# beecave-homelab/VibeVoice-ROCm

Measured on AMD Instinct MI355X. Metric: audio-sec/s, higher is better.
Workload: dtype bf16; 1 GPU; cfg2: VibeVoice-1.5B shapes, 1 speaker(s) x 203-frame voice prompt, 330-token prompt, 225 frames (30.0 s audio), CFG=2.0, 20 DPM-Solver++ steps, whole generate() incl. voice encode + prefill; global_batch=1, parallelism=replicas x1 (one dialogue per GPU), hipgraph=True

## Files before the change

include/vv_hip.h:

```cpp
#ifndef VV_HIP_H
#define VV_HIP_H

#include <stddef.h>
#include <stdint.h>

#ifdef __cplusplus
extern "C" {
#endif

typedef void* vv_stream_t;

enum { VV_F32 = 0, VV_BF16 = 1, VV_FP8 = 2  };
enum { VV_NF4 = 3 };
enum { VV_WQ_NF4 = 0x100 };
enum { VV_OK = 0, VV_E_ARG = -1, VV_E_HIP = -2, VV_E_UNSUPPORTED = -3 };
enum { VV_PRO_NONE = 0, VV_PRO_RMSNORM = 1, VV_PRO_SILU = 2 };
enum { VV_ACT_NONE = 0, VV_ACT_GELU = 1, VV_ACT_SWIGLU = 2 };
enum { VV_LIN_X_BF16 = 1, VV_LIN_OUT_BF16 = 2, VV_LIN_W_REUSED = 4, VV_LIN_W_FRAG = 8 };

const char* vv_last_error(void);
int vv_abi_version(void);
int vv_tune(const char* key, int value);
int vv_init(void);

// ... 154 lines not shown

size_t vv_block_mid_ws_bytes(int T, int C);
int vv_block_mid(const struct vv_block* b, int wdt, const float* x, float* out, void* ws, int T, int C, float eps, vv_stream_t stream);

typedef struct vv_conv {
  const void* w;
  const float* b;
  int cin, cout, kk, stride, transposed;
  float* state;
} vv_conv;

#define VV_MAX_STAGES 8
typedef struct vv_convnet {
  int wdt, n_stages;
  float eps;
  vv_conv sample[VV_MAX_STAGES];
  int n_blocks[VV_MAX_STAGES];
  const vv_block* blocks[VV_MAX_STAGES];
  vv_conv head;
} vv_convnet;

size_t vv_convnet_ws_bytes(const vv_convnet* net, int64_t t_in, int decoder);
int vv_decoder_forward(const vv_convnet* net, const float* latent, int T, float pre_scale, float pre_bias, float* wav,
                       void* ws, vv_stream_t stream);
int vv_encoder_forward(const vv_convnet* net, const float* wav, int64_t T, float* feat, void* ws, vv_stream_t stream);
int vv_convnet_reset(const vv_convnet* net, vv_stream_t stream);

typedef struct vv_connector { int wdt, din, hidden; const void* fc1; const float* b1; const float* norm_w; const void* fc2; const float* b2; } vv_connector;
int vv_connector_forward(const vv_connector* c, const float* x, int R, float* out, int accumulate, float* ws, vv_stream_t stream);
int vv_connector_pair(const vv_connector* ac, const vv_connector* sem, const float* latent, const float* semfeat, float* out, int64_t ldo,
                      int rows_out, float* ws, vv_stream_t stream);

int vv_graph_begin(vv_stream_t stream);
int vv_graph_end(vv_stream_t stream, void** graph_exec_out);
int vv_graph_launch(void* graph_exec, vv_stream_t stream);
int vv_graph_destroy(void* graph_exec);

typedef struct vv_prof_entry { int m, n, k, dual, wdt, count; double total_ms; } vv_prof_entry;
int vv_prof_begin(int max_records);
int vv_prof_end(vv_prof_entry* out, int max_out, int* n_out);

typedef struct vv_nf4_src {
  const uint8_t* packed;
  const void* absmax;
  const float* quant_map;
  const float* nested_absmax;
  const float* nested_map;
  float nested_offset;
  int nested_blocksize;
  int n, k, blocksize;
} vv_nf4_src;
int vv_nf4_import(const vv_nf4_src* src, void* w, int64_t ldw, int row0, int rows_total, void* cq, float* cs, vv_stream_t stream);

size_t vv_sizeof(const char* struct_name);

#ifdef __cplusplus
}
#endif
#endif
```

vibevoice_rocm_amd/_lib.py:

```python
from __future__ import annotations

import ctypes as C
import os

_HERE = os.path.dirname(os.path.abspath(__file__))
LIB_PATH = os.path.join(_HERE, "libvv_hip.so")

VV_F32, VV_BF16, VV_FP8, VV_NF4 = 0, 1, 2, 3
VV_WQ_NF4 = 0x100
PRO_NONE, PRO_RMSNORM, PRO_SILU = 0, 1, 2
ACT_NONE, ACT_GELU, ACT_SWIGLU = 0, 1, 2
LIN_X_BF16, LIN_OUT_BF16, LIN_W_REUSED, LIN_W_FRAG = 1, 2, 4, 8
VV_MAX_STAGES = 8

vp = C.c_void_p
i64 = C.c_int64


class W8(C.Structure):
    _fields_ = [("q", vp), ("scale", vp)]


class LinArgs(C.Structure):
    _fields_ = [("x", vp), ("ldx", i64), ("m", C.c_int), ("pro", C.c_int), ("norm_w", vp), ("eps", C.c_float),
# ... 68 lines not shown
_STRUCTS = dict(vv_w8=W8, vv_prof_entry=ProfEntry, vv_lin_args=LinArgs, vv_kv=KV, vv_llm_layer=LlmLayer, vv_llm=Llm, vv_head_layer=HeadLayer, vv_head=Head,
                vv_dpm_coef=DpmCoef, vv_block=Block, vv_conv=Conv, vv_convnet=ConvNet, vv_connector=Connector, vv_nf4_src=Nf4Src)

PROTOTYPES = {
    "vv_last_error": (C.c_char_p, []),
    "vv_abi_version": (C.c_int, []),
    "vv_init": (C.c_int, []),
    "vv_tune": (C.c_int, [C.c_char_p, C.c_int]),
    "vv_linear": (C.c_int, [C.POINTER(LinArgs), vp]),
    "vv_rope_table": (C.c_int, [vp, vp, C.c_int, C.c_int, vp, vp]),
    "vv_rope_store": (C.c_int, [vp, i64, C.c_int, C.c_int, C.POINTER(KV), C.c_int, vp, vp, vp, vp]),
    "vv_attn": (C.c_int, [vp, i64, C.c_int, C.c_int, C.POINTER(KV), C.c_int, vp, vp, vp, i64, vp]),
    "vv_attn_decode": (C.c_int, [vp, i64, C.c_int, C.c_int, C.POINTER(KV), C.c_int, vp, vp, vp, i64, vp]),
    "vv_block_mixer": (C.c_int, [vp, vp, C.c_int, C.c_int, vp, C.c_float, vp, vp, vp, vp, vp]),
    "vv_block1d": (C.c_int, [vp, C.c_int, vp, vp, C.c_int, C.c_int, C.c_float, vp]),
    "vv_block_mid_ws_bytes": (C.c_size_t, [C.c_int, C.c_int]),
    "vv_block_mid": (C.c_int, [vp, C.c_int, vp, vp, vp, C.c_int, C.c_int, C.c_float, vp]),
    "vv_conv_ctx": (C.c_int, [vp, vp, C.c_int, C.c_int, C.c_int, vp]),
    "vv_affine": (C.c_int, [vp, C.c_float, C.c_float, vp, i64, vp]),
    "vv_add_rows": (C.c_int, [vp, i64, vp, i64, vp, C.c_int, C.c_int, C.c_int, vp]),
    "vv_add_rows_silu": (C.c_int, [vp, i64, vp, i64, vp, C.c_int, C.c_int, C.c_int, vp]),
    "vv_add_rows_silu_bf16": (C.c_int, [vp, i64, vp, i64, vp, C.c_int, C.c_int, C.c_int, vp]),
    "vv_dpm_proj": (C.c_int, [vp, i64, C.c_float, C.POINTER(DpmCoef), vp, vp, vp, vp, vp, C.c_int, C.c_int, C.c_int, vp, i64, C.c_int, vp, vp]),
    "vv_embed_row": (C.c_int, [vp, C.c_int, i64, vp, vp, vp]),
    "vv_gather_rows": (C.c_int, [vp, C.c_int, i64, C.POINTER(C.c_int), C.c_int, vp, vp]),
    "vv_argmax_ids": (C.c_int, [vp, C.c_int, vp, vp, vp, vp]),
    "vv_cast_rows_bf16": (C.c_int, [vp, i64, C.c_int, C.c_int, C.c_int, vp, C.c_float, vp, i64, vp]),
    "vv_copy_rows": (C.c_int, [vp, i64, vp, i64, C.c_int, C.c_int, vp]),
    "vv_dpm_step": (C.c_int, [vp, i64, C.c_int, C.c_int, C.c_float, C.c_float, C.c_float, C.c_float, C.c_float,
                              C.c_float, C.c_int, vp, vp, vp]),
    "vv_advance_lens": (C.c_int, [vp, vp, C.c_int, C.c_int, vp, vp]),
    "vv_llm_ws_bytes": (C.c_size_t, [C.POINTER(Llm), C.c_int]),
    "vv_llm_forward": (C.c_int, [C.POINTER(Llm), C.POINTER(KV), vp, i64, C.c_int, vp, vp, vp, i64, vp, vp]),
    "vv_llm_tail": (C.c_int, [C.POINTER(Llm), vp, i64, C.c_int, vp, i64, vp, C.c_int, vp, vp, vp, vp, vp, C.c_int, C.c_int, vp, vp]),
    "vv_llm_tail_batch": (C.c_int, [C.POINTER(Llm), vp, i64, C.c_int, vp, i64, vp, C.c_int, vp, vp, vp, vp, vp, C.c_int, C.c_int, vp, vp, vp]),
    "vv_head_ws_bytes": (C.c_size_t, [C.POINTER(Head), C.c_int]),
    "vv_head_ws_bytes_batch": (C.c_size_t, [C.POINTER(Head), C.c_int, C.c_int]),
    "vv_head_sample_batch": (C.c_int, [C.POINTER(Head), vp, i64, vp, i64, vp, C.POINTER(DpmCoef), C.c_int, C.c_float, vp, i64, C.c_int, vp, vp]),
    "vv_head_ws_bytes_batch_sde": (C.c_size_t, [C.POINTER(Head), C.c_int, C.c_int]),
    "vv_head_sample_batch_sde": (C.c_int, [C.POINTER(Head), vp, i64, vp, i64, vp, C.POINTER(DpmCoef), C.c_int, C.c_float, vp, i64, C.c_int, vp, vp, i64, vp]),
    "vv_head_sample": (C.c_int, [C.POINTER(Head), vp, i64, vp, vp, C.POINTER(DpmCoef), C.c_int, C.c_float, vp, vp, vp, vp]),
    "vv_head_forward": (C.c_int, [C.POINTER(Head), vp, vp, vp, C.c_int, vp, vp, vp]),
    "vv_convnet_ws_bytes": (C.c_size_t, [C.POINTER(ConvNet), i64, C.c_int]),
    "vv_decoder_forward": (C.c_int, [C.POINTER(ConvNet), vp, C.c_int, C.c_float, C.c_float, vp, vp, vp]),
    "vv_encoder_forward": (C.c_int, [C.POINTER(ConvNet), vp, i64, vp, vp, vp]),
    "vv_convnet_reset": (C.c_int, [C.POINTER(ConvNet), vp]),
    "vv_connector_forward": (C.c_int, [C.POINTER(Connector), vp, C.c_int, vp, C.c_int, vp, vp]),
    "vv_connector_pair": (C.c_int, [C.POINTER(Connector), C.POINTER(Connector), vp, vp, vp, i64, C.c_int, vp, vp]),
    "vv_graph_begin": (C.c_int, [vp]),
    "vv_graph_end": (C.c_int, [vp, C.POINTER(vp)]),
    "vv_graph_launch": (C.c_int, [vp, vp]),
    "vv_graph_destroy": (C.c_int, [vp]),
    "vv_nf4_import": (C.c_int, [C.POINTER(Nf4Src), vp, i64, C.c_int, C.c_int, vp, vp, vp]),
    "vv_sizeof": (C.c_size_t, [C.c_char_p]),
    "vv_prof_begin": (C.c_int, [C.c_int]),
    "vv_prof_end": (C.c_int, [C.POINTER(ProfEntry), C.c_int, C.POINTER(C.c_int)]),
}


class VVError(RuntimeError):
    pass


_lib = None


def load():
    global _lib
    if _lib is not None:
        return _lib
    import torch
    if not os.path.exists(LIB_PATH):
        raise VVError(f"{LIB_PATH} is missing: build the HIP extension first (python -m vibevoice_rocm_amd.build). "
                      "The MI355X kernels are the only compute path of this package.")
    lib = C.CDLL(LIB_PATH)
    for name, (res, args) in PROTOTYPES.items():
        fn = getattr(lib, name)
        fn.restype = res
        fn.argtypes = args
    for cname, cls in _STRUCTS.items():
        n = lib.vv_sizeof(cname.encode())
        if n != C.sizeof(cls):
            raise VVError(f"ABI mismatch for {cname}: C side {n} bytes, ctypes mirror {C.sizeof(cls)} bytes")
    _lib = lib
    return lib


def check(rc: int, what: str = ""):
    if rc != 0:
        raise VVError(f"{what} failed ({rc}): {load().vv_last_error().decode()}")


def ptr(t) -> int:
    return 0 if t is None else t.data_ptr()
```

vibevoice_rocm_amd/build.py:

```python
from __future__ import annotations

import hashlib
import os
import shutil
import subprocess
import sys

HERE = os.path.dirname(os.path.abspath(__file__))
ROOT = os.path.dirname(HERE)
SRC = [os.path.join(HERE, "csrc", f) for f in ("vv_kernels.hip", "vv_gemv_stream.hip", "vv_gemv_hot.hip", "vv_gemv_rows.hip", "vv_mfma_gemm.hip", "vv_block1d.hip", "vv_convffn.hip",
                                               "vv_fused.hip", "vv_attn_decode.hip", "vv_attn_prefill.hip", "vv_model.hip",
                                               "vv_nf4_import.hip")]
HDR = [os.path.join(ROOT, "include", "vv_hip.h"), os.path.join(HERE, "csrc", "vv_common.h")]
OUT = os.path.join(HERE, "libvv_hip.so")
OBJDIR = os.path.join(HERE, "csrc", "build")
STAMP = os.path.join(HERE, "libvv_hip.stamp")
FLAGS = ["--offload-arch=gfx950", "-O3", "-std=c++17", "-fPIC"]


def find_hipcc() -> str:
    for c in (os.environ.get("HIPCC"), shutil.which("hipcc"), "/opt/rocm/bin/hipcc"):
        if c and os.path.exists(c):
            return c
    raise RuntimeError("hipcc not found (ROCm toolchain required to build the MI355X kernels)")


def _flavour() -> str:
    return hashlib.sha256("\n".join([os.path.basename(s) for s in SRC] + FLAGS).encode()).hexdigest()[:16]


def _check_sources():
    missing = [p for p in SRC + HDR if not os.path.exists(p)]
    if missing:
        raise RuntimeError("missing kernel sources: " + ", ".join(os.path.relpath(p, ROOT) for p in missing))


def up_to_date() -> bool:
    if not os.path.exists(OUT):
        return False
    if not all(os.path.exists(p) for p in SRC + HDR):
        return True
    t = os.path.getmtime(OUT)
    if not all(os.path.getmtime(p) <= t for p in SRC + HDR):
        return False
    try:
        return open(STAMP).read().strip() == _flavour()
    except OSError:
        return False


def _obj(src: str) -> str:
    return os.path.join(OBJDIR, os.path.basename(src) + ".o")


def build(force: bool = False, verbose: bool = True, jobs: int = 6) -> str:
    if not force and up_to_date():
        return OUT
    _check_sources()
    os.makedirs(OBJDIR, exist_ok=True)
    flags = [*FLAGS, "-I" + os.path.join(ROOT, "include"), "-I" + os.path.join(HERE, "csrc")]
    hipcc = find_hipcc()
    hdr_t = max(os.path.getmtime(p) for p in HDR)
    todo = [s for s in SRC if force or not os.path.exists(_obj(s)) or os.path.getmtime(_obj(s)) < max(os.path.getmtime(s), hdr_t)]
# ... 24 lines not shown
```

vibevoice_rocm_amd/csrc/vv_common.h:

```cpp
#ifndef VV_COMMON_H
#define VV_COMMON_H
#include <hip/hip_runtime.h>
#include <stdarg.h>
#include <stdint.h>
#include "vv_hip.h"

int vv_set_error(int code, const char* fmt, ...);

#define VV_CHECK_LAUNCH(name)                                                                    \
  do {                                                                                           \
    hipError_t e_ = hipGetLastError();                                                           \
    if (e_ != hipSuccess) return vv_set_error(VV_E_HIP, "%s: %s", name, hipGetErrorString(e_));  \
  } while (0)

#define VV_TRY(expr)            \
  do {                          \
    int rc_ = (expr);           \
    if (rc_) return rc_;        \
  } while (0)

int vv_launch_gemv_stream(const vv_lin_args& a, hipStream_t s);
struct vv_gemv_hot_shape { const char* name; int m, n, k, dual, pro, mod, bias, gate, res, act, flags; };
extern "C" int vv_gemv_hot_shapes(vv_gemv_hot_shape* out, int cap);
int vv_launch_gemv_hot(const vv_lin_args& a, hipStream_t s);
void vv_gemv_hot_set(int mask);
int vv_launch_gemv_rows(const vv_lin_args& a, float* part, size_t part_floats, int* tickets, size_t n_tickets, hipStream_t s);
size_t vv_gemv_rows_part_floats(int n, int dual);
size_t vv_gemv_rows_tickets(int n);
int vv_gemv_rows_init();
void vv_gemv_rows_set(int on, int blocks, int pers);
int vv_linear_ws(const vv_lin_args* a, const void* f1, const void* f2, float* part, size_t part_floats, int* tickets, size_t n_tickets,
                 vv_stream_t stream, const vv_w8* q1 = nullptr, const vv_w8* q2 = nullptr);
int vv_launch_mfma_gemm(const vv_lin_args& a, hipStream_t s);
int vv_mfma_gemm_init();
int vv_launch_attn_decode(const float* qkv, int64_t ld_qkv, int R, int heads, const vv_kv* kv, int layer, const float2* rope, const int* lens, float* out,
                          int64_t ldo, float* part, int* tickets, int nsplit, int part_cap, hipStream_t s);
int vv_attn_decode_ws(const float* qkv, int64_t ld_qkv, int R, int heads, const vv_kv* kv, int layer, const float* rope_table, const int* lens, float* out,
                      int64_t ldo, float* part, int* tickets, int nsplit, int part_cap, vv_stream_t stream);
int vv_launch_attn_prefill(const float* qkv, int64_t ld_qkv, int R, int heads, const vv_kv* kv, int layer, const int* lens, const int* cache_rows,
                           float* out, int64_t ldo, hipStream_t s);
int vv_head_init_fused(const vv_head* h, const float* noise, float* Xs, float* Ms, float* h0, int64_t ldh, hipStream_t s);
bool vv_head_boundary_supported(const vv_head* h);
int vv_head_boundary_fused(const vv_head* h, const float* hrows, int64_t ldh, const float* shift, const float* scale, int64_t ld_mod, float cfg,
                           const vv_dpm_coef* k, float* Xs, float* Ms, float* h_out, int64_t ldh_out, float* latent_out, hipStream_t s);
int vv_head_boundary_batch(const vv_head* h, const float* hrows, int64_t ldh, const float* shift, const float* scale, int64_t ld_mod, float cfg,
                           const vv_dpm_coef* k, float* Xs, float* Ms, int64_t state_stride, float* h_out, int64_t ldh_out, float* latent_out,
                           int64_t latent_stride, int B, hipStream_t s,
                           const float* nx = nullptr, int64_t nx_stride = 0);
int vv_head_sde_proj_fused(const vv_head* h, const float* sde_noise, int64_t ld_sde, int n_steps, int B, float* NX, hipStream_t s);
int vv_fused_init();
int vv_head_pre_fused(const vv_head* h, const float* cond2, int64_t ld_cond, const float* temb, int n_steps, void* c_bf16, const float* noise,
                      float* Xs, float* Ms, float* h0, int64_t ldh, hipStream_t s);
int vv_launch_connector_pair(const vv_connector* ac, const vv_connector* sem, const float* latent, const float* semfeat, float* out, int64_t ldo, int rows_out,
                             float* ws, hipStream_t s);
int vv_head_modulations_fused(const vv_head* h, const void* c_bf16, int rows, float* const* mod, float* modf, hipStream_t s);
struct vv_conv_ctx_item { float* pad; float* state; int ctx, T, C; const float* dw_w; float* hs; int affine; float scale, bias; };
int vv_conv_ctx_batch(const vv_conv_ctx_item* items, int n, int scatter, hipStream_t s);
int vv_block1d_init();
int vv_launch_block1d(const vv_block& B, int wdt, const float* x, float* out, int T, int C, float eps, hipStream_t s);
void vv_block1d_set_fused(int on);
void vv_block1d_set_blocks(int b);
int vv_convffn_init();
int vv_launch_convffn(const vv_block& B, int wdt, const float* x, float* y, void* hidden, float* hist_new, float* out, int T, int C, float eps,
                      hipStream_t s);
void vv_convffn_set(int on);
int vv_launch_ffn_in_row(const vv_block& B, int wdt, const float* x, float* y, float* hidden, float* hist_new, int C, float eps, hipStream_t s);
void vv_convffn_set_t1(int on);
int vv_launch_ffn_in_row_hs(const vv_block& B, int wdt, const float* x, float* y, float* hidden, float* hist_new, int C, float eps, hipStream_t s);
void vv_convffn_set_t1hs(int on);
void vv_convffn_set_rows(int c, int rows);
void vv_convffn_set_c128(int on);
bool vv_convffn_prefers(int wdt, int T, int C);
int vv_launch_skinny(const vv_lin_args& a, hipStream_t s);
void vv_skinny_set(int on, int min_m, int max_m);
int vv_rmsnorm_rows(const float* x, int64_t ldx, const float* w, float eps, int rows, int n, float* out, int64_t ldo, hipStream_t s);

#ifdef __HIPCC__
__device__ __forceinline__ float vv_gelu_as(float v) {
// ... 24 lines not shown
```

vibevoice_rocm_amd/csrc/vv_convffn.hip:

```cpp
#include <hip/hip_runtime.h>
#include <hip/hip_bf16.h>
#include <stdint.h>

#include "vv_hip.h"
#include "vv_common.h"

namespace {

typedef unsigned short bf16_t;
typedef __bf16 bf16x8 __attribute__((ext_vector_type(8)));
typedef float f32x16 __attribute__((ext_vector_type(16)));
typedef float f32x4 __attribute__((ext_vector_type(4)));
typedef unsigned int u32x4 __attribute__((ext_vector_type(4)));

#ifdef VV_CF_TIMING
__device__ unsigned long long g_cf_t[8];
#define CSTAMP(i) do { if (blockIdx.x == 0 && blockIdx.y == 0 && threadIdx.x == 0) { const long long t_ = wall_clock64(); g_cf_t[i] += (unsigned long long)(t_ - tprev_); tprev_ = t_; } } while (0)
#else
#define CSTAMP(i) do { } while (0)
#endif

constexpr int TR2 = 16;
constexpr int HALO = 6;

// ... 494 lines not shown
#define VV_SK(NSTV, NBV) hipLaunchKernelGGL((skinny_kernel<NSTV, NBV>), grid, dim3(256), 0, s, a.x, a.ldx, a.m, W, a.k, a.bias, a.out, a.ldo)
  switch (a.k) {
    case 128: VV_SK(1, 1); break;
    case 256: VV_SK(2, 1); break;
    case 512: VV_SK(4, 1); break;
    case 1024: VV_SK(8, 1); break;
    case 2048: VV_SK(16, 1); break;
    case 2560: VV_SK(20, 1); break;
    case 5120: VV_SK(20, 2); break;
    default: return 0;
  }
#undef VV_SK
  return 1;
}

int vv_convffn_init() {
#define VV_CF_ATTR(CC, TT)                                                                                                                  \
  { constexpr int nt_ = in_threads<CC>(); constexpr int l_ = (int)InLay<CC, TT, nt_>::LDS;                                                 \
    if (hipFuncSetAttribute(reinterpret_cast<const void*>(&ffn_in_kernel<CC, TT, false, nt_>), hipFuncAttributeMaxDynamicSharedMemorySize, l_) != hipSuccess) \
      return vv_set_error(VV_E_HIP, "vv_convffn_init: cannot raise the LDS limit"); }
  VV_CF_ATTR(128, 16) VV_CF_ATTR(128, 32) VV_CF_ATTR(256, 8) VV_CF_ATTR(256, 16) VV_CF_ATTR(256, 32) VV_CF_ATTR(512, 8) VV_CF_ATTR(512, 16) VV_CF_ATTR(512, 32) VV_CF_ATTR(1024, 8)
#undef VV_CF_ATTR
  {
    constexpr int l1 = (int)InLay<2048, 1, 256>::LDS;
    if (hipFuncSetAttribute(reinterpret_cast<const void*>(&ffn_in_kernel<2048, 1, true, 256>), hipFuncAttributeMaxDynamicSharedMemorySize, l1) != hipSuccess)
      return vv_set_error(VV_E_HIP, "vv_convffn_init: cannot raise the LDS limit");
  }
  return 0;
}

int g_t1 = 1;
void vv_convffn_set_t1(int on) { g_t1 = on; }

int vv_launch_ffn_in_row(const vv_block& B, int wdt, const float* x, float* y, float* hidden, float* hist_new, int C, float eps, hipStream_t s) {
  if (!g_on || !g_t1 || wdt != VV_BF16 || C != 2048 || !B.hist) return 0;
  auto a16 = [](const void* q) { return q && ((uintptr_t)q % 16) == 0; };
  if (!a16(B.w1) || !a16(B.b1) || !a16(B.gamma) || !a16(B.norm_w) || !a16(B.ffn_norm_w) || !a16(B.dw_b) || !a16(B.dw_w) || !a16(x) || !a16(y) ||
      !a16(hidden) || !a16(hist_new) || !a16(B.hist) || x == y)
    return 0;
  constexpr size_t lds = InLay<2048, 1, 256>::LDS;
  hipLaunchKernelGGL((ffn_in_kernel<2048, 1, true, 256>), dim3(4 * 2048 / 32, 1), dim3(256), lds, s, x, y, hidden, hist_new, 1, B, eps);
  return hipGetLastError() == hipSuccess ? 1 : vv_set_error(VV_E_HIP, "vv_convffn: launch failed");
}

int g_t1hs = 1;
void vv_convffn_set_t1hs(int on) { g_t1hs = on; }

int vv_launch_ffn_in_row_hs(const vv_block& B, int wdt, const float* x, float* y, float* hidden, float* hist_new, int C, float eps, hipStream_t s) {
  if (!g_on || !g_t1 || !g_t1hs || wdt != VV_BF16 || C != 2048 || !B.hist || !B.hs || !B.dw_last) return 0;
  auto a16 = [](const void* q) { return q && ((uintptr_t)q % 16) == 0; };
  if (!a16(B.w1) || !a16(B.b1) || !a16(B.gamma) || !a16(B.norm_w) || !a16(B.ffn_norm_w) || !a16(B.dw_b) || !a16(B.dw_last) || !a16(B.hs) || !a16(x) ||
      !a16(y) || !a16(hidden) || !a16(hist_new) || !a16(B.hist) || x == y)
    return 0;
  hipLaunchKernelGGL(ffn_in_row_kernel, dim3(4 * 2048 / 32), dim3(256), 0, s, x, y, hidden, hist_new, B, eps);
  return hipGetLastError() == hipSuccess ? 1 : vv_set_error(VV_E_HIP, "vv_convffn: launch failed");
}

int vv_launch_convffn(const vv_block& B, int wdt, const float* x, float* y, void* hidden, float* hist_new, float* out, int T, int C, float eps,
                      hipStream_t s) {
  if (!g_on || wdt != VV_BF16 || T < 3 || (C != 128 && C != 256 && C != 512 && C != 1024) || (C == 1024 && T > 64)) return 0;
  if (C == 128 ? (!g_c128 || T > 1024) : T > 256) return 0;
  auto a16 = [](const void* q) { return q && ((uintptr_t)q % 16) == 0; };
  if (!a16(B.w1) || !a16(B.w2) || !a16(B.b1) || !B.b2 || !a16(B.gamma) || !B.ffn_gamma || !a16(B.norm_w) || !a16(B.ffn_norm_w) || !a16(B.dw_b) ||
      !a16(B.dw_w) || !a16(x) || !a16(y) || !a16(hidden) || !a16(hist_new) || !out || (B.hist && !a16(B.hist)))
    return 0;
  {
    const uintptr_t xa = (uintptr_t)x, ya = (uintptr_t)y, bytes = (uintptr_t)T * C * 4;
    if (xa < ya + bytes && ya < xa + bytes) return 0;
  }
  if (C == 128) {
    if (g_trv128 == 16) return launch_c<128, 16, 4>(B, x, y, hidden, hist_new, out, T, eps, s);
    return launch_c<128, 32, 4>(B, x, y, hidden, hist_new, out, T, eps, s);
  }
  if (C == 256) {
    if (g_trv256 == 8) return launch_c<256, 8, 4>(B, x, y, hidden, hist_new, out, T, eps, s);
    if (g_trv256 == 16) return launch_c<256, 16, 4>(B, x, y, hidden, hist_new, out, T, eps, s);
    return launch_c<256, 32, 4>(B, x, y, hidden, hist_new, out, T, eps, s);
  }
  if (C == 512) {
    if (g_trv512 == 8) return launch_c<512, 8, 4>(B, x, y, hidden, hist_new, out, T, eps, s);
    if (g_trv512 == 16) return launch_c<512, 16, 4>(B, x, y, hidden, hist_new, out, T, eps, s);
    return launch_c<512, 32, 4>(B, x, y, hidden, hist_new, out, T, eps, s);
  }
  return launch_c<1024, 8, 8>(B, x, y, hidden, hist_new, out, T, eps, s);
}

extern "C" size_t vv_block_mid_ws_bytes(int T, int C) { return (size_t)T * C * 4 + (size_t)T * 4 * C * 2 + (size_t)HALO * C * 4 + 64; }

extern "C" int vv_block_mid(const vv_block* b, int wdt, const float* x, float* out, void* ws, int T, int C, float eps, vv_stream_t stream) {
  if (!b || !x || !out || !ws || T <= 0) return vv_set_error(VV_E_ARG, "vv_block_mid: bad args");
  float* y = reinterpret_cast<float*>(ws);
  char* hidden = reinterpret_cast<char*>(ws) + (size_t)T * C * 4;
  float* hn = reinterpret_cast<float*>(hidden + (size_t)T * 4 * C * 2);
  const int rc = vv_launch_convffn(*b, wdt, x, y, hidden, hn, out, T, C, eps, (hipStream_t)stream);
  if (rc < 0) return rc;
  if (rc == 0) return vv_set_error(VV_E_UNSUPPORTED, "vv_block_mid: shape not covered (C=%d T=%d wdt=%d)", C, T, wdt);
  return 0;
}
```

vibevoice_rocm_amd/csrc/vv_gemv_stream.hip:

```cpp
#include <hip/hip_runtime.h>
#include <stdint.h>

#include "vv_hip.h"
#include "vv_common.h"

namespace {

typedef unsigned short bf16_t;
typedef unsigned int u32x4 __attribute__((ext_vector_type(4)));

__device__ __forceinline__ float wsum(float v) { return vv_wave_sum(v); }
__device__ __forceinline__ float silu1(float v) { return v / (1.0f + expf(-v)); }
__device__ __forceinline__ float gelu1(float v) { return 0.5f * v * (1.0f + erff(v * 0.70710678118654752440f)); }

__device__ __forceinline__ void unpack8(const u32x4 v, float (&o)[8]) {
  o[0] = __uint_as_float(v.x << 16); o[1] = __uint_as_float(v.x & 0xffff0000u);
  o[2] = __uint_as_float(v.y << 16); o[3] = __uint_as_float(v.y & 0xffff0000u);
  o[4] = __uint_as_float(v.z << 16); o[5] = __uint_as_float(v.z & 0xffff0000u);
  o[6] = __uint_as_float(v.w << 16); o[7] = __uint_as_float(v.w & 0xffff0000u);
}

typedef unsigned int u32x2 __attribute__((ext_vector_type(2)));
typedef float f32x2 __attribute__((ext_vector_type(2)));
__device__ __forceinline__ void unpack8_f8(const u32x4 v, float (&o)[8]) {
// ... 551 lines not shown
    case 8: return launch_kus<M, DUAL, 8>(a, s, ku);
    case 16: if constexpr (!DUAL) return launch_kus<M, false, 16>(a, s, ku); else return false;
  }
  return false;
}

bool launch_m8(const vv_lin_args& a, hipStream_t s, int ksplit, int ku) {
  if (ksplit == 1) {
    if (ku == 1) launch_rw<8, false, 1, 1, 1>(a, s); else launch_rw<8, false, 1, 2, 1>(a, s);
    return true;
  }
  switch (ksplit) {
    case 4: launch_rw<8, false, 4, 2, 2>(a, s); return true;
    case 8: launch_rw<8, false, 8, 2, 2>(a, s); return true;
  }
  return false;
}

}

void vv_gemv_stream_set_blocks(int b) { g_blocks_override = b; }
void vv_gemv_stream_set_waves(int w) { g_waves_override = w; }
void vv_gemv_stream_set_opt(int o) { g_opt = o; }
void vv_gemv_stream_set_long(int cap, int ku) { if (cap > 0) g_long_cap = cap; if (ku > 0) g_long_ku = ku; }
void vv_gemv_stream_set_dual_rw(int r) { g_dual_rw = r; }
void vv_gemv_stream_set_small_rw(int r) { g_small_rw = r; }

int vv_launch_gemv_stream(const vv_lin_args& a, hipStream_t s) {
  if ((a.wdt != VV_BF16 && a.wdt != VV_FP8 && a.wdt != VV_NF4) || a.m > 8 || a.k % 8) return 0;
  if (a.wdt == VV_NF4 && (a.m > 2 || a.k % 64 || !a.wscale || (a.w2 && !a.w2scale) || (uintptr_t)a.w % 16 || (a.w2 && (uintptr_t)a.w2 % 16) ||
                          (uintptr_t)a.wscale % 4 || (a.w2 && (uintptr_t)a.w2scale % 4) || (a.flags & VV_LIN_W_FRAG)))
    return 0;
  if (a.wdt == VV_FP8 && (a.m > 2 || !a.wscale || (a.w2 && !a.w2scale) || (uintptr_t)a.w % 8 || (a.w2 && (uintptr_t)a.w2 % 8))) return 0;
  if (a.m > 4) {
    if (a.w2 || a.wdt != VV_BF16) return 0;
    if ((uintptr_t)a.w % 16 || (uintptr_t)a.x % 16 || a.ldx % 4) return 0;
    if (a.norm_w && (uintptr_t)a.norm_w % 16) return 0;
    if (a.mod_scale && ((uintptr_t)a.mod_scale % 16 || (uintptr_t)a.mod_shift % 16 || a.ld_mod % 4)) return 0;
    const int units8 = (a.k + 511) / 512;
    int ks = 0, ku8 = 0;
    for (int w : {1, 4, 8}) {
      if ((units8 + w - 1) / w <= 2) { ks = w; ku8 = (units8 + w - 1) / w; break; }
    }
    if (!ks) return 0;
    if (ks > 1) ku8 = 2;
    return launch_m8(a, s, ks, ku8) ? 1 : 0;
  }
  if (a.wdt == VV_BF16 && ((uintptr_t)a.w % 16 || (a.w2 && (uintptr_t)a.w2 % 16))) return 0;
  if ((uintptr_t)a.x % 16) return 0;
  if (a.m > 1 && a.ldx % 4) return 0;
  if (a.norm_w && (uintptr_t)a.norm_w % 16) return 0;
  if (a.mod_scale && ((uintptr_t)a.mod_scale % 16 || (uintptr_t)a.mod_shift % 16 || a.ld_mod % 4)) return 0;
  if (a.m == 2 && a.wdt == VV_BF16 && vv_launch_gemv_hot(a, s)) return 1;
  const int units = (a.k + 511) / 512;
  const bool dual = a.w2 != nullptr;
  int ksplit = 1, ku = units;
  if (units > ((a.wdt == VV_NF4 && dual) ? 4 : 5)) {
    const int kumax = dual ? 3 : (units > 12 ? g_long_ku : 5);
    ksplit = 0;
    for (int w : {4, 8, 16}) {
      if ((units + w - 1) / w <= kumax) { ksplit = w; ku = (units + w - 1) / w; break; }
    }
    if (!ksplit) return 0;
    if (ku < 2) ku = 2;
  }
  if (a.wdt == VV_NF4 && ksplit > 8) return 0;
  bool ok;
  if (a.m == 1) ok = dual ? launch_ku<1, true>(a, s, ksplit, ku) : launch_ku<1, false>(a, s, ksplit, ku);
  else if (a.m == 2) ok = dual ? launch_ku<2, true>(a, s, ksplit, ku) : launch_ku<2, false>(a, s, ksplit, ku);
  else ok = dual ? launch_ku<4, true>(a, s, ksplit, ku) : launch_ku<4, false>(a, s, ksplit, ku);
  return ok ? 1 : 0;
}
```

vibevoice_rocm_amd/csrc/vv_kernels.hip:

```cpp
#include <hip/hip_runtime.h>
#include <hip/hip_bf16.h>
#include <stdint.h>
#include <stdio.h>
#include <string.h>
#include <math.h>

#include "vv_hip.h"
#include "vv_common.h"

static thread_local char g_err[512] = "";

int vv_set_error(int code, const char* fmt, ...) {
  va_list ap;
  va_start(ap, fmt);
  vsnprintf(g_err, sizeof(g_err), fmt, ap);
  va_end(ap);
  return code;
}

extern "C" const char* vv_last_error(void) { return g_err; }
extern "C" int vv_abi_version(void) { return 6; }
int vv_mixer_init();
extern "C" int vv_init(void) {
  VV_TRY(vv_mixer_init());
  VV_TRY(vv_mfma_gemm_init());
  VV_TRY(vv_block1d_init());
  VV_TRY(vv_convffn_init());
  VV_TRY(vv_gemv_rows_init());
  return vv_fused_init();
}
static float* g_rows_part = nullptr;
static int* g_rows_tk = nullptr;
static const size_t G_ROWS_PART_FLOATS = (size_t)4 << 20, G_ROWS_TICKETS = 4096;
static int rows_scratch(int on) {
  if (on && !g_rows_part) {
    if (hipMalloc(&g_rows_part, G_ROWS_PART_FLOATS * sizeof(float)) != hipSuccess || hipMalloc(&g_rows_tk, G_ROWS_TICKETS * sizeof(int)) != hipSuccess ||
        hipMemset(g_rows_tk, 0, G_ROWS_TICKETS * sizeof(int)) != hipSuccess)
      return vv_set_error(VV_E_HIP, "vv_tune: gemv_rows_scratch allocation failed");
  }
  if (!on && g_rows_part) { (void)hipFree(g_rows_part); (void)hipFree(g_rows_tk); g_rows_part = nullptr; g_rows_tk = nullptr; }
  return 0;
}
void vv_gemv_rows_set_dbg(int d);
void vv_gemv_rows_set_atomic(int on);
void vv_gemv_stream_set_blocks(int b);
void vv_gemv_stream_set_waves(int w);
void vv_gemv_stream_set_opt(int o);
void vv_gemv_stream_set_long(int cap, int ku);
void vv_gemv_stream_set_dual_rw(int r);
void vv_gemv_stream_set_small_rw(int r);
void vv_mfma_set_mt(int mt);
void vv_mfma_set_tiled_rows(int r);
void vv_mfma_set_tiled_bk128(int on);
void vv_mfma_set_tiled_small(int t);
void vv_mfma_set_tiled_dual_bk64(int on);
void vv_mfma_set_tiled_small_dual(int t);
void vv_mfma_set_tiled_small_k(int k);
void vv_mixer_set_rows(int on);
void vv_mfma_set_mt_prefill(int mt);
extern int g_attn_group;
void vv_attn_decode_set_gqa(int on);
void vv_attn_decode_set_gqa_keys(int k);
extern "C" int vv_tune(const char* key, int value) {
  if (key && !strcmp(key, "gemv_long_cap")) { vv_gemv_stream_set_long(value, 0); return 0; }
  if (key && !strcmp(key, "gemv_long_ku")) { vv_gemv_stream_set_long(0, value); return 0; }
  if (key && !strcmp(key, "gemv_blocks")) { vv_gemv_stream_set_blocks(value); return 0; }
  if (key && !strcmp(key, "gemv_waves")) { vv_gemv_stream_set_waves(value); return 0; }
  if (key && !strcmp(key, "gemv_rows")) { vv_gemv_rows_set(value, 0, -1); return 0; }
  if (key && !strcmp(key, "gemv_rows_blocks")) { vv_gemv_rows_set(-1, value, -1); return 0; }
  if (key && !strcmp(key, "gemv_rows_pers")) { vv_gemv_rows_set(-1, 0, value); return 0; }
  if (key && !strcmp(key, "gemv_rows_scratch")) return rows_scratch(value);
  if (key && !strcmp(key, "gemv_rows_dbg")) { vv_gemv_rows_set_dbg(value); return 0; }
  if (key && !strcmp(key, "gemv_rows_atomic")) { vv_gemv_rows_set_atomic(value); return 0; }
  if (key && !strcmp(key, "gemv_opt")) { vv_gemv_stream_set_opt(value); return 0; }
  if (key && !strcmp(key, "gemv_dual_rw")) { vv_gemv_stream_set_dual_rw(value); return 0; }
  if (key && !strcmp(key, "gemv_small_rw")) { vv_gemv_stream_set_small_rw(value); return 0; }
  if (key && !strcmp(key, "gemv_hot")) { vv_gemv_hot_set(value); return 0; }
  if (key && !strcmp(key, "mixer_rows")) { vv_mixer_set_rows(value); return 0; }
  if (key && !strcmp(key, "block1d_fused")) { vv_block1d_set_fused(value); return 0; }
  if (key && !strcmp(key, "block1d_blocks")) { vv_block1d_set_blocks(value); return 0; }
  if (key && !strcmp(key, "convffn")) { vv_convffn_set(value); return 0; }
  if (key && !strcmp(key, "convffn_t1")) { vv_convffn_set_t1(value); return 0; }
  if (key && !strcmp(key, "convffn_t1hs")) { vv_convffn_set_t1hs(value); return 0; }
  if (key && !strcmp(key, "convffn_rows512")) { vv_convffn_set_rows(512, value); return 0; }
  if (key && !strcmp(key, "convffn_rows256")) { vv_convffn_set_rows(256, value); return 0; }
  if (key && !strcmp(key, "convffn_rows128")) { vv_convffn_set_rows(128, value); return 0; }
  if (key && !strcmp(key, "convffn_c128")) { vv_convffn_set_c128(value); return 0; }
  if (key && !strcmp(key, "skinny")) { vv_skinny_set(value, 0, 0); return 0; }
  if (key && !strcmp(key, "skinny_min_m")) { vv_skinny_set(1, value, 0); return 0; }
  if (key && !strcmp(key, "skinny_max_m")) { vv_skinny_set(1, 0, value); return 0; }
  if (key && !strcmp(key, "mfma_tiled_bk128")) { vv_mfma_set_tiled_bk128(value); return 0; }
  if (key && !strcmp(key, "attn_group")) { g_attn_group = value; return 0; }
  if (key && !strcmp(key, "attn_gqa")) { vv_attn_decode_set_gqa(value); return 0; }
  if (key && !strcmp(key, "attn_gqa_keys")) { vv_attn_decode_set_gqa_keys(value); return 0; }
  if (key && !strcmp(key, "mfma_tiled_small_k")) { vv_mfma_set_tiled_small_k(value); return 0; }
  if (key && !strcmp(key, "mfma_tiled_dual_bk64")) { vv_mfma_set_tiled_dual_bk64(value); return 0; }
  if (key && !strcmp(key, "mfma_tiled_small_dual")) { vv_mfma_set_tiled_small_dual(value); return 0; }
  if (key && !strcmp(key, "mfma_tiled_small")) { vv_mfma_set_tiled_small(value); return 0; }
  if (key && !strcmp(key, "mfma_tiled_rows")) { vv_mfma_set_tiled_rows(value); return 0; }
  if (key && !strcmp(key, "mfma_mt")) { vv_mfma_set_mt(value); return 0; }
  if (key && !strcmp(key, "mfma_mt_prefill")) { vv_mfma_set_mt_prefill(value); return 0; }
  return vv_set_error(VV_E_ARG, "vv_tune: unknown key");
}

typedef unsigned short bf16_t;

__device__ __forceinline__ float bf2f(unsigned int u16) { return __uint_as_float(u16 << 16); }
__device__ __forceinline__ float wave_sum(float v) {
#pragma unroll
  for (int o = 32; o > 0; o >>= 1) v += __shfl_xor(v, o);
  return v;
}
__device__ __forceinline__ float wave_sum_dpp(float v) { return vv_wave_sum(v); }
__device__ __forceinline__ float silu_f(float v) { return v / (1.0f + expf(-v)); }
__device__ __forceinline__ float gelu_f(float v) { return 0.5f * v * (1.0f + erff(v * 0.70710678118654752440f)); }

template <typename WT> struct WL;
template <> struct WL<float> {
  static __device__ __forceinline__ void load8(const float* p, float (&o)[8]) {
    const float4 a = *reinterpret_cast<const float4*>(p);
    const float4 b = *reinterpret_cast<const float4*>(p + 4);
    o[0] = a.x; o[1] = a.y; o[2] = a.z; o[3] = a.w; o[4] = b.x; o[5] = b.y; o[6] = b.z; o[7] = b.w;
  }
  static __device__ __forceinline__ void load4(const float* p, float (&o)[4]) {
    const float4 a = *reinterpret_cast<const float4*>(p);
    o[0] = a.x; o[1] = a.y; o[2] = a.z; o[3] = a.w;
  }
  static __device__ __forceinline__ float load1(const float* p) { return *p; }
};
template <> struct WL<bf16_t> {
// ... 1577 lines not shown
```

Baseline: 42.25 audio-sec/s.

## Add shape-specialized hot kernels for conv-block GEMVs and FFN input row

Adds a new source file with compile-time specialized m=1 bf16 GEMV kernels for the conv block w2 and the decoder/semantic handover projections. These kernels issue every weight load up front (nontemporal) with fused bias/gate/residual. It also adds an MFMA-based replacement for the fused RMSNorm+depthwise+FFN-input row kernel, which computes history rows in an extra workgroup. Both are on by default and dispatched before the generic stream GEMV and the old row kernel. The aim is to cut latency of memory-bound single-token conv-decoder matvecs, at the cost of more code and very high register pressure in the fully unrolled loads.

```diff
diff --git a/include/vv_hip.h b/include/vv_hip.h
--- a/include/vv_hip.h
+++ b/include/vv_hip.h
@@ -230,6 +230,11 @@
 } vv_nf4_src;
 int vv_nf4_import(const vv_nf4_src* src, void* w, int64_t ldw, int row0, int rows_total, void* cq, float* cs, vv_stream_t stream);
 
+#define VV_CONV_HOT_GEMV 0
+#define VV_CONV_HOT_ROW 1
+typedef struct vv_conv_hot_shape { const char* name; int kind, m, n, k, bias, gate, res; } vv_conv_hot_shape;
+int vv_conv_hot_shapes(vv_conv_hot_shape* out, int cap);
+
 size_t vv_sizeof(const char* struct_name);
 
 #ifdef __cplusplus
diff --git a/vibevoice_rocm_amd/_lib.py b/vibevoice_rocm_amd/_lib.py
--- a/vibevoice_rocm_amd/_lib.py
+++ b/vibevoice_rocm_amd/_lib.py
@@ -144,6 +144,7 @@
     "vv_graph_launch": (C.c_int, [vp, vp]),
     "vv_graph_destroy": (C.c_int, [vp]),
     "vv_nf4_import": (C.c_int, [C.POINTER(Nf4Src), vp, i64, C.c_int, C.c_int, vp, vp, vp]),
+    "vv_conv_hot_shapes": (C.c_int, [vp, C.c_int]),
     "vv_sizeof": (C.c_size_t, [C.c_char_p]),
     "vv_prof_begin": (C.c_int, [C.c_int]),
     "vv_prof_end": (C.c_int, [C.POINTER(ProfEntry), C.c_int, C.POINTER(C.c_int)]),
diff --git a/vibevoice_rocm_amd/build.py b/vibevoice_rocm_amd/build.py
--- a/vibevoice_rocm_amd/build.py
+++ b/vibevoice_rocm_amd/build.py
@@ -8,7 +8,7 @@
 
 HERE = os.path.dirname(os.path.abspath(__file__))
 ROOT = os.path.dirname(HERE)
-SRC = [os.path.join(HERE, "csrc", f) for f in ("vv_kernels.hip", "vv_gemv_stream.hip", "vv_gemv_hot.hip", "vv_gemv_rows.hip", "vv_mfma_gemm.hip", "vv_block1d.hip", "vv_convffn.hip",
+SRC = [os.path.join(HERE, "csrc", f) for f in ("vv_kernels.hip", "vv_gemv_stream.hip", "vv_gemv_hot.hip", "vv_conv_hot.hip", "vv_gemv_rows.hip", "vv_mfma_gemm.hip", "vv_block1d.hip", "vv_convffn.hip",
                                                "vv_fused.hip", "vv_attn_decode.hip", "vv_attn_prefill.hip", "vv_model.hip",
                                                "vv_nf4_import.hip")]
 HDR = [os.path.join(ROOT, "include", "vv_hip.h"), os.path.join(HERE, "csrc", "vv_common.h")]
diff --git a/vibevoice_rocm_amd/csrc/vv_common.h b/vibevoice_rocm_amd/csrc/vv_common.h
--- a/vibevoice_rocm_amd/csrc/vv_common.h
+++ b/vibevoice_rocm_amd/csrc/vv_common.h
@@ -24,6 +24,9 @@
 extern "C" int vv_gemv_hot_shapes(vv_gemv_hot_shape* out, int cap);
 int vv_launch_gemv_hot(const vv_lin_args& a, hipStream_t s);
 void vv_gemv_hot_set(int mask);
+int vv_launch_conv_hot_gemv(const vv_lin_args& a, hipStream_t s);
+int vv_launch_conv_hot_row(const vv_block& B, const float* x, float* y, float* hidden, float* hist_new, int C, float eps, hipStream_t s);
+void vv_conv_hot_set(int mask);
 int vv_launch_gemv_rows(const vv_lin_args& a, float* part, size_t part_floats, int* tickets, size_t n_tickets, hipStream_t s);
 size_t vv_gemv_rows_part_floats(int n, int dual);
 size_t vv_gemv_rows_tickets(int n);
diff --git a/vibevoice_rocm_amd/csrc/vv_conv_hot.hip b/vibevoice_rocm_amd/csrc/vv_conv_hot.hip
--- /dev/null
+++ b/vibevoice_rocm_amd/csrc/vv_conv_hot.hip
@@ -0,0 +1,300 @@
+#include <hip/hip_runtime.h>
+#include <hip/hip_bf16.h>
+#include <stdint.h>
+
+#include "vv_hip.h"
+#include "vv_common.h"
+
+namespace {
+
+typedef unsigned short bf16_t;
+typedef unsigned int u32x4 __attribute__((ext_vector_type(4)));
+typedef float vf2 __attribute__((ext_vector_type(2)));
+typedef __bf16 bf16x8 __attribute__((ext_vector_type(8)));
+typedef float f32x16 __attribute__((ext_vector_type(16)));
+
+__device__ __forceinline__ void unpack8(const u32x4 v, float (&o)[8]) {
+  o[0] = __uint_as_float(v.x << 16); o[1] = __uint_as_float(v.x & 0xffff0000u);
+  o[2] = __uint_as_float(v.y << 16); o[3] = __uint_as_float(v.y & 0xffff0000u);
+  o[4] = __uint_as_float(v.z << 16); o[5] = __uint_as_float(v.z & 0xffff0000u);
+  o[6] = __uint_as_float(v.w << 16); o[7] = __uint_as_float(v.w & 0xffff0000u);
+}
+
+template <bool NT>
+__device__ __forceinline__ u32x4 ldw(const bf16_t* p) {
+  const u32x4* q = reinterpret_cast<const u32x4*>(p);
+  if constexpr (NT) return __builtin_nontemporal_load(q);
+  else return *q;
+}
+
+__device__ __forceinline__ void fma_unit(const u32x4 wv, const float (&x)[8], vf2& p) {
+  float w[8];
+  unpack8(wv, w);
+#pragma unroll
+  for (int j = 0; j < 8; j += 2) p = __builtin_elementwise_fma(vf2{w[j], w[j + 1]}, vf2{x[j], x[j + 1]}, p);
+}
+
+__device__ __forceinline__ float gate_res(float v, float g, float r) {
+#pragma clang fp contract(off)
+  const float t = v * g;
+  return t + r;
+}
+
+#define VV_FENCE4(v) asm volatile("" : "+v"((v).x), "+v"((v).y), "+v"((v).z), "+v"((v).w))
+
+template <int N, int K, int NW, int R, bool GR>
+__global__ __launch_bounds__(64 * NW) void conv_gemv_kernel(const vv_lin_args a) {
+  constexpr int KU = K / (512 * NW);
+  static_assert(K % (512 * NW) == 0 && N % R == 0 && R <= 64 && R * KU + 2 * KU + 3 < 63, "whole units, whole row sets, every load in flight at once");
+  __shared__ float part[NW][R];
+  const int tid = threadIdx.x, lane = tid & 63;
+  const int wave = __builtin_amdgcn_readfirstlane(tid >> 6);
+  const int n0 = (int)blockIdx.x * R;
+  const bf16_t* __restrict__ W = reinterpret_cast<const bf16_t*>(a.w);
+
+  int koff[KU];
+#pragma unroll
+  for (int u = 0; u < KU; ++u) koff[u] = (wave + NW * u) * 512 + lane * 8;
+  float4 xa[KU], xb[KU];
+#pragma unroll
+  for (int u = 0; u < KU; ++u) {
+    xa[u] = *reinterpret_cast<const float4*>(a.x + koff[u]);
+    xb[u] = *reinterpret_cast<const float4*>(a.x + koff[u] + 4);
+  }
+  const int eo_n = n0 + (tid < R ? tid : 0);
+  const float eb = a.bias[eo_n];
+  float eg = 1.f, er = 0.f;
+  if constexpr (GR) { eg = a.gate[eo_n]; er = a.res[eo_n]; }
+  u32x4 wq[R][KU];
+#pragma unroll
+  for (int r = 0; r < R; ++r)
+#pragma unroll
+    for (int u = 0; u < KU; ++u) wq[r][u] = ldw<true>(W + (n0 + r) * K + koff[u]);
+  __builtin_amdgcn_sched_barrier(0);
+#pragma unroll
+  for (int u = 0; u < KU; ++u) { VV_FENCE4(xa[u]); VV_FENCE4(xb[u]); }
+
+  float xr[KU][8];
+#pragma unroll
+  for (int u = 0; u < KU; ++u) {
+    xr[u][0] = xa[u].x; xr[u][1] = xa[u].y; xr[u][2] = xa[u].z; xr[u][3] = xa[u].w;
+    xr[u][4] = xb[u].x; xr[u][5] = xb[u].y; xr[u][6] = xb[u].z; xr[u][7] = xb[u].w;
+  }
+  float acc[R];
+#pragma unroll
+  for (int r = 0; r < R; ++r) {
+    vf2 p = vf2{0.f, 0.f};
+#pragma unroll
+    for (int u = 0; u < KU; ++u) fma_unit(wq[r][u], xr[u], p);
+    acc[r] = vv_wave_sum(p.x + p.y);
+  }
+  if (lane == 0) {
+#pragma unroll
+    for (int r = 0; r < R; ++r) part[wave][r] = acc[r];
+  }
+  __syncthreads();
+  if (tid < R) {
+    float s = 0.f;
+#pragma unroll
+    for (int w4 = 0; w4 < NW; ++w4) s += part[w4][tid];
+    float v = s + eb;
+    if constexpr (GR) v = gate_res(v, eg, er);
+    a.out[eo_n] = v;
+  }
+}
+
+__device__ __forceinline__ unsigned int pack2(float a, float b) {
+  const __hip_bfloat16 x = __float2bfloat16(a), y = __float2bfloat16(b);
+  return (unsigned int)(*reinterpret_cast<const bf16_t*>(&x)) | ((unsigned int)(*reinterpret_cast<const bf16_t*>(&y)) << 16);
+}
+__device__ __forceinline__ void ld4(const float* p, float (&o)[4]) {
+  const float4 t = *reinterpret_cast<const float4*>(p);
+  o[0] = t.x; o[1] = t.y; o[2] = t.z; o[3] = t.w;
+}
+__device__ __forceinline__ void st4(float* p, const float (&o)[4]) { *reinterpret_cast<float4*>(p) = make_float4(o[0], o[1], o[2], o[3]); }
+
+constexpr int ROW_C = 2048, ROW_WG = 4 * ROW_C / 32;
+
+template <bool NT>
+__global__ __launch_bounds__(256) void row_in_kernel(const float* __restrict__ x, float* __restrict__ y, float* __restrict__ hidden,
+                                                     float* __restrict__ hist_new, const vv_block B, float eps) {
+  constexpr int C = ROW_C, P1 = C + 8, ST = C / 64;
+  __shared__ __attribute__((aligned(16))) bf16_t xh[P1];
+  __shared__ float red[4 * 16 * 2];
+  __shared__ float part[8];
+  const int tid = threadIdx.x, lane = tid & 63, wave = __builtin_amdgcn_readfirstlane(tid >> 6);
+  int c0[2];
+#pragma unroll
+  for (int j = 0; j < 2; ++j) c0[j] = 4 * (tid + 256 * j);
+
+  if (blockIdx.x == ROW_WG) {
+    float xv[2][4], nw[2][4], hrow[5][2][4];
+#pragma unroll
+    for (int j = 0; j < 2; ++j) {
+      ld4(x + c0[j], xv[j]);
+      ld4(B.norm_w + c0[j], nw[j]);
+    }
+#pragma unroll
+    for (int r = 0; r < 5; ++r)
+#pragma unroll
+      for (int j = 0; j < 2; ++j) ld4(B.hist + (size_t)(r + 1) * C + c0[j], hrow[r][j]);
+    float q = 0.f;
+#pragma unroll
+    for (int j = 0; j < 2; ++j)
+#pragma unroll
+      for (int e = 0; e < 4; ++e) q = fmaf(xv[j][e], xv[j][e], q);
+    q = vv_wave_sum(q);
+    if (lane == 0) part[wave] = q;
+    __syncthreads();
+    const float rstd1 = rsqrtf(((part[0] + part[1]) + (part[2] + part[3])) / (float)C + eps);
+#pragma unroll
+    for (int j = 0; j < 2; ++j) {
+      float xn[4];
+#pragma unroll
+      for (int e = 0; e < 4; ++e) xn[e] = xv[j][e] * rstd1 * nw[j][e];
+#pragma unroll
+      for (int r = 0; r < 5; ++r) st4(hist_new + (size_t)r * C + c0[j], hrow[r][j]);
+      st4(hist_new + (size_t)5 * C + c0[j], xn);
+    }
+    return;
+  }
+
+  const int n0 = blockIdx.x * 32;
+  const int lm = lane & 31, hk = (lane >> 5) * 8;
+  float xv[2][4], hsv[2][4], dl[2][4], nw[2][4], db[2][4], gm[2][4], fw[2][4];
+#pragma unroll
+  for (int j = 0; j < 2; ++j) {
+    ld4(x + c0[j], xv[j]);
+    ld4(B.norm_w + c0[j], nw[j]);
+    ld4(B.hs + c0[j], hsv[j]);
+    ld4(B.dw_last + c0[j], dl[j]);
+    ld4(B.dw_b + c0[j], db[j]);
+    ld4(B.gamma + c0[j], gm[j]);
+    ld4(B.ffn_norm_w + c0[j], fw[j]);
+  }
+  u32x4 wf[ST];
+  {
+    const bf16_t* wr = reinterpret_cast<const bf16_t*>(B.w1) + (int64_t)(n0 + lm) * C + wave * (C / 4) + hk;
+#pragma unroll
+    for (int s = 0; s < ST; ++s) wf[s] = ldw<NT>(wr + s * 16);
+  }
+  const float b1v = B.b1[n0 + lm];
+  __builtin_amdgcn_sched_barrier(0);
+  float q = 0.f;
+#pragma unroll
+  for (int j = 0; j < 2; ++j)
+#pragma unroll
+    for (int e = 0; e < 4; ++e) q = fmaf(xv[j][e], xv[j][e], q);
+  q = vv_wave_sum(q);
+  if (lane == 0) part[wave] = q;
+  __syncthreads();
+  const float rstd1 = rsqrtf(((part[0] + part[1]) + (part[2] + part[3])) / (float)C + eps);
+  float yv[2][4], xn[2][4];
+  float q2 = 0.f;
+#pragma unroll
+  for (int j = 0; j < 2; ++j)
+#pragma unroll
+    for (int e = 0; e < 4; ++e) {
+      xn[j][e] = xv[j][e] * rstd1 * nw[j][e];
+      const float sc = db[j][e] + hsv[j][e] + dl[j][e] * xn[j][e];
+      yv[j][e] = xv[j][e] + gm[j][e] * sc;
+      q2 = fmaf(yv[j][e], yv[j][e], q2);
+    }
+  q2 = vv_wave_sum(q2);
+  if (lane == 0) part[4 + wave] = q2;
+  __syncthreads();
+  const float rstd2 = rsqrtf(((part[4] + part[5]) + (part[6] + part[7])) / (float)C + eps);
+  {
+    const int ys0 = blockIdx.x * (C / ROW_WG);
+#pragma unroll
+    for (int j = 0; j < 2; ++j) {
+      uint2 p;
+      p.x = pack2(yv[j][0] * rstd2 * fw[j][0], yv[j][1] * rstd2 * fw[j][1]);
+      p.y = pack2(yv[j][2] * rstd2 * fw[j][2], yv[j][3] * rstd2 * fw[j][3]);
+      *reinterpret_cast<uint2*>(xh + c0[j]) = p;
+      if (c0[j] >= ys0 && c0[j] < ys0 + C / ROW_WG) st4(y + c0[j], yv[j]);
+    }
+  }
+  __syncthreads();
+  f32x16 acc;
+#pragma unroll
+  for (int i = 0; i < 16; ++i) acc[i] = 0.f;
+  {
+    const bf16_t* xf = xh + wave * (C / 4) + hk;
+#pragma unroll
+    for (int s = 0; s < ST; ++s) {
+      const u32x4 xb = *reinterpret_cast<const u32x4*>(xf + s * 16);
+      acc = __builtin_amdgcn_mfma_f32_32x32x16_bf16(__builtin_bit_cast(bf16x8, wf[s]), __builtin_bit_cast(bf16x8, xb), acc, 0, 0, 0);
+    }
+  }
+  if (lm == 0) {
+#pragma unroll
+    for (int r = 0; r < 16; ++r) red[(wave * 16 + r) * 2 + (lane >> 5)] = acc[r];
+  }
+  __syncthreads();
+  if (tid < 32) {
+    const int r = 4 * (tid >> 3) + (tid & 3), h = (tid >> 2) & 1;
+    float s = 0.f;
+#pragma unroll
+    for (int w4 = 0; w4 < 4; ++w4) s += red[(w4 * 16 + r) * 2 + h];
+    hidden[n0 + tid] = vv_gelu_as(s + b1v);
+  }
+}
+
+#undef VV_FENCE4
+
+constexpr int N_HOT = 4;
+const vv_conv_hot_shape g_table[N_HOT] = {
+    {"block.w2",         VV_CONV_HOT_GEMV, 1, 2048, 8192,  1,   1,   1},
+    {"block.ffn_in_row", VV_CONV_HOT_ROW,  1, 8192, 2048,  1,   0,   0},
+    {"dec.handover",     VV_CONV_HOT_GEMV, 1, 8192, 4096,  1,   0,   0},
+    {"sem.handover",     VV_CONV_HOT_GEMV, 1, 2048, 16384, 1,   0,   0},
+};
+
+constexpr int HOT_DEFAULT = 0xf;
+int g_hot = HOT_DEFAULT;
+
+bool matches(const vv_conv_hot_shape& e, const vv_lin_args& a) {
+  return e.kind == VV_CONV_HOT_GEMV && a.m == e.m && a.n == e.n && a.k == e.k && a.wdt == VV_BF16 && !a.w2 && a.pro == VV_PRO_NONE && !a.mod_scale &&
+         !a.mod_shift && (a.bias != nullptr) == (e.bias != 0) && (a.gate != nullptr) == (e.gate != 0) && (!e.gate || a.gate_ld == 0) &&
+         (a.res != nullptr) == (e.res != 0) && a.act == VV_ACT_NONE && a.flags == 0;
+}
+
+}
+
+void vv_conv_hot_set(int mask) { g_hot = mask < 0 ? HOT_DEFAULT : mask; }
+
+extern "C" int vv_conv_hot_shapes(vv_conv_hot_shape* out, int cap) {
+  for (int i = 0; i < N_HOT && i < cap; ++i) out[i] = g_table[i];
+  return N_HOT;
+}
+
+int vv_launch_conv_hot_gemv(const vv_lin_args& a, hipStream_t s) {
+  if (!(g_hot & ((1 << N_HOT) - 1)) || a.m != 1 || a.wdt != VV_BF16) return 0;
+  int id = -1;
+  for (int i = 0; i < N_HOT; ++i)
+    if ((g_hot >> i & 1) && matches(g_table[i], a)) { id = i; break; }
+  const bool alt = (g_hot & 256) != 0;
+  switch (id) {
+    case 0:
+      if (alt) hipLaunchKernelGGL((conv_gemv_kernel<2048, 8192, 4, 4, true>), dim3(512), dim3(256), 0, s, a);
+      else hipLaunchKernelGGL((conv_gemv_kernel<2048, 8192, 4, 8, true>), dim3(256), dim3(256), 0, s, a);
+      return 1;
+    case 2:
+      if (alt) hipLaunchKernelGGL((conv_gemv_kernel<8192, 4096, 4, 16, false>), dim3(512), dim3(256), 0, s, a);
+      else hipLaunchKernelGGL((conv_gemv_kernel<8192, 4096, 4, 8, false>), dim3(1024), dim3(256), 0, s, a);
+      return 1;
+    case 3:
+      if (alt) hipLaunchKernelGGL((conv_gemv_kernel<2048, 16384, 8, 8, false>), dim3(256), dim3(512), 0, s, a);
+      else hipLaunchKernelGGL((conv_gemv_kernel<2048, 16384, 8, 4, false>), dim3(512), dim3(512), 0, s, a);
+      return 1;
+  }
+  return 0;
+}
+
+int vv_launch_conv_hot_row(const vv_block& B, const float* x, float* y, float* hidden, float* hist_new, int C, float eps, hipStream_t s) {
+  if (!(g_hot & 2) || C != ROW_C || !hist_new) return 0;
+  if (!(g_hot & 512)) hipLaunchKernelGGL(row_in_kernel<false>, dim3(ROW_WG + 1), dim3(256), 0, s, x, y, hidden, hist_new, B, eps);
+  else hipLaunchKernelGGL(row_in_kernel<true>, dim3(ROW_WG + 1), dim3(256), 0, s, x, y, hidden, hist_new, B, eps);
+  return 1;
+}
diff --git a/vibevoice_rocm_amd/csrc/vv_convffn.hip b/vibevoice_rocm_amd/csrc/vv_convffn.hip
--- a/vibevoice_rocm_amd/csrc/vv_convffn.hip
+++ b/vibevoice_rocm_amd/csrc/vv_convffn.hip
@@ -570,7 +570,8 @@
   if (!a16(B.w1) || !a16(B.b1) || !a16(B.gamma) || !a16(B.norm_w) || !a16(B.ffn_norm_w) || !a16(B.dw_b) || !a16(B.dw_last) || !a16(B.hs) || !a16(x) ||
       !a16(y) || !a16(hidden) || !a16(hist_new) || !a16(B.hist) || x == y)
     return 0;
-  hipLaunchKernelGGL(ffn_in_row_kernel, dim3(4 * 2048 / 32), dim3(256), 0, s, x, y, hidden, hist_new, B, eps);
+  if (!vv_launch_conv_hot_row(B, x, y, hidden, hist_new, C, eps, s))
+    hipLaunchKernelGGL(ffn_in_row_kernel, dim3(4 * 2048 / 32), dim3(256), 0, s, x, y, hidden, hist_new, B, eps);
   return hipGetLastError() == hipSuccess ? 1 : vv_set_error(VV_E_HIP, "vv_convffn: launch failed");
 }
 
diff --git a/vibevoice_rocm_amd/csrc/vv_gemv_stream.hip b/vibevoice_rocm_amd/csrc/vv_gemv_stream.hip
--- a/vibevoice_rocm_amd/csrc/vv_gemv_stream.hip
+++ b/vibevoice_rocm_amd/csrc/vv_gemv_stream.hip
@@ -627,6 +627,7 @@
   if (a.norm_w && (uintptr_t)a.norm_w % 16) return 0;
   if (a.mod_scale && ((uintptr_t)a.mod_scale % 16 || (uintptr_t)a.mod_shift % 16 || a.ld_mod % 4)) return 0;
   if (a.m == 2 && a.wdt == VV_BF16 && vv_launch_gemv_hot(a, s)) return 1;
+  if (a.m == 1 && a.wdt == VV_BF16 && vv_launch_conv_hot_gemv(a, s)) return 1;
   const int units = (a.k + 511) / 512;
   const bool dual = a.w2 != nullptr;
   int ksplit = 1, ku = units;
diff --git a/vibevoice_rocm_amd/csrc/vv_kernels.hip b/vibevoice_rocm_amd/csrc/vv_kernels.hip
--- a/vibevoice_rocm_amd/csrc/vv_kernels.hip
+++ b/vibevoice_rocm_amd/csrc/vv_kernels.hip
@@ -76,6 +76,7 @@
   if (key && !strcmp(key, "gemv_dual_rw")) { vv_gemv_stream_set_dual_rw(value); return 0; }
   if (key && !strcmp(key, "gemv_small_rw")) { vv_gemv_stream_set_small_rw(value); return 0; }
   if (key && !strcmp(key, "gemv_hot")) { vv_gemv_hot_set(value); return 0; }
+  if (key && !strcmp(key, "conv_hot")) { vv_conv_hot_set(value); return 0; }
   if (key && !strcmp(key, "mixer_rows")) { vv_mixer_set_rows(value); return 0; }
   if (key && !strcmp(key, "block1d_fused")) { vv_block1d_set_fused(value); return 0; }
   if (key && !strcmp(key, "block1d_blocks")) { vv_block1d_set_blocks(value); return 0; }
```

Measured after the change: 42.88 audio-sec/s, median of 6. +1.5%, better.
